# TigreGotico/phoonnx

Hardware: AMD Instinct MI355X
Metric: audio samples/sec (22.05 kHz), batch-32 256-phoneme utterances (higher is better)
Workload: dtype f32 (f16x3 split: fp32 operands as two fp16 planes, three MFMA products, fp32 accumulate)

## Files before the change

### include/vitsmi.h

```cpp
#ifndef VITSMI_H
#define VITSMI_H

#include <stddef.h>
#include <stdint.h>

#ifdef __cplusplus
extern "C" {
#endif

typedef struct vits_handle vits_handle;

enum {
    VITS_OK = 0,
    VITS_E_IO = -1,
    VITS_E_FORMAT = -2,
    VITS_E_ARG = -3,
    VITS_E_DEVICE = -4,
    VITS_E_NOMEM = -5,
    VITS_E_RANGE = -6
};

#define VITS_MAX_DIMS 4


// ... 192 lines not shown
    int cin, cout, k, dil, t;
} vits_launch_record;
int vits_launch_records(vits_handle *h, vits_launch_record *buf, int n);

void *vits_stream(vits_handle *h);


int vits_test_conv1d(int device_id, const float *x, int B, int Cin, int T, const float *w, const float *bias,
                     int Cout, int K, int dil, int pad_l, int flags, float slope, float *out);
int vits_bench_conv1d(int device_id, int B, int Cin, int Cout, int T, int K, int dil, int hint, int iters,
                      int cfg_override, int ck_override, float *ms_out);
int vits_test_conv_transpose1d(int device_id, const float *x, int B, int Cin, int T, const float *w,
                               const float *bias, int Cout, int K, int stride, float *out);
int vits_test_conv1d_sx(int device_id, const float *x, int B, int Cin, int T, const float *w, const float *bias,
                        int Cout, int K, int dil, int pad_l, int flags, float slope, float *out);
int vits_test_conv1d_sx_planar(int device_id, const float *x, int B, int Cin, int T, const float *w, const float *bias,
                               int Cout, int K, int dil, int flags, const int64_t *lens, const float *old, int row_split,
                               int pl_rows, float *out, float *planes_out);
long long vits_test_set_sx_small_max(long long wgs);
int vits_test_conv1d_sx_gate(int device_id, const float *x, int B, int Cin, int T, const float *w, const float *bias,
                             const float *bias_b, int Cout, int K, int dil, int flags, float *out);
int vits_test_conv_transpose1d_sx(int device_id, const float *x, int B, int Cin, int T, const float *w,
                                  const float *bias, int Cout, int K, int stride, float *out);
int vits_bench_conv1d_sx(int device_id, int B, int Cin, int Cout, int T, int K, int dil, int dbg, int iters,
                         float *ms_out);
int vits_test_conv_pair_sx(int device_id, const float *x, int B, int C, int T, const float *w1, const float *b1,
                           const float *w2, const float *b2, int K, int dil1, int dil2, int chain, float slope, float *out,
                           float *ms_out);
int vits_test_attention(int device_id, const float *qkv, int B, int C, int T, int n_heads, const float *rel_k,
                        const float *rel_v, int window, const int64_t *lens, float *out);
int vits_test_attention16(int device_id, const float *qkv, int B, int C, int T, int n_heads, const float *rel_k,
                          const float *rel_v, int window, const int64_t *lens, float *out, uint16_t *out_planes, int kernel,
                          int reps, float *ms_out);

int vits_test_resample(int device_id, const float *x, const int64_t *lens, int B, int S, int in_rate, int out_rate, float *y,
                       int64_t S_out);
int vits_test_resample_pieces(int device_id, const float *x, const int64_t *lens, int B, int S, int in_rate, int out_rate,
                              int piece_samples, float *y, int64_t S_out, int64_t *ranges, int max_ranges);

int vits_test_durations(int device_id, const float *logw, const int64_t *dur, const int64_t *lens, int B, int T, float length_scale,
                        const float *rows, const float *token_rate, float *w_ceil, int32_t *cum, int32_t *y_len);
int vits_test_expand_prior(int device_id, const float *m_logs, int B, int C, int T, const int32_t *cum, const int64_t *lens,
                           const int32_t *y_len, int F, const float *noise, int64_t noise_stride, int noise_frames,
                           float noise_scale, const float *rows, const uint64_t *seeds, float *z_p);
int vits_test_fill_normal(int device_id, int64_t n, uint64_t seed, uint64_t stream_id, float *out);
int vits_test_fill_normal_rows(int device_id, int B, int channels, int T, const uint64_t *seeds, uint32_t stream, const float *rows,
// ... 47 lines not shown
```

### phoonnx_amd/_ffi.py

```python
import ctypes as C
import os

import numpy as np

from . import audio_encoding

_HERE = os.path.dirname(os.path.abspath(__file__))
_LIB = None

VITS_MAX_DIMS = 4


class VitsNoise(C.Structure):
    _fields_ = [("noise_dp", C.c_void_p), ("noise_z", C.c_void_p), ("noise_z_stride", C.c_int64),
                ("seed", C.c_uint64)]


class VitsOutput(C.Structure):
    _fields_ = [("data", C.POINTER(C.c_float)), ("dims", C.c_int64 * 4), ("y_lengths", C.POINTER(C.c_int64))]


class VitsStats(C.Structure):
    _fields_ = [("conv_flops", C.c_double), ("conv_bytes", C.c_double), ("dec_flops", C.c_double),
                ("dec_bytes", C.c_double), ("flow_flops", C.c_double), ("enc_flops", C.c_double),
# ... 40 lines not shown
class VitsStreamFormat(C.Structure):
    _fields_ = [("encoding", C.c_int32), ("ref_peak", C.c_void_p), ("volume", C.c_void_p)]


ENCODINGS = {name: (code, audio_encoding.DTYPES[name]) for code, name in enumerate(audio_encoding.ENCODINGS)}


CHUNK_FN = C.CFUNCTYPE(C.c_int, C.c_void_p, C.POINTER(C.c_float), C.c_int, C.c_int64, C.c_int64, C.c_int64)

ENC_CHUNK_FN = C.CFUNCTYPE(C.c_int, C.c_void_p, C.c_void_p, C.c_int, C.c_int64, C.c_int64, C.c_int64, C.POINTER(C.c_int32),
                           C.POINTER(C.c_float), C.c_int64)

VITS_E_RANGE = -6


EXPORTS = [
    "vits_open", "vits_open_with_arena", "vits_open_host", "vits_open_layout", "vits_open_opts", "vits_close",
    "vits_run_chunked", "vits_run_vocoder_chunked", "vits_last_error", "vits_num_inputs",
    "vits_input_name", "vits_meta", "vits_hparam", "vits_arena_bytes", "vits_arena_host", "vits_arena_device",
    "vits_run", "vits_free_output", "vits_run_device", "vits_sync", "vits_last_y_lengths", "vits_last_pcm16", "vits_run_vocoder",
    "vits_tap",
    "vits_set_timing", "vits_set_tails", "vits_reserve", "vits_get_stats", "vits_stream", "vits_test_conv1d", "vits_test_conv_transpose1d",
    "vits_test_attention", "vits_test_attention16", "vits_bench_conv1d", "vits_test_conv1d_sx", "vits_test_conv1d_sx_planar", "vits_test_conv1d_sx_gate", "vits_test_set_sx_small_max",
    "vits_test_conv_transpose1d_sx",
    "vits_bench_conv1d_sx", "vits_test_conv_pair_sx", "vits_fetch_output", "vits_run_async", "vits_host_alloc", "vits_host_free",
    "vits_launch_records", "vits_run_async_rows", "vits_run_device_rows", "vits_run_chunked_rows",
    "vits_run_async_ctl", "vits_run_chunked_ctl", "vits_last_durations",
    "vits_set_output_rate", "vits_last_sample_counts", "vits_resample_plan", "vits_test_resample", "vits_test_resample_pieces",
    "vits_test_durations", "vits_test_expand_prior", "vits_test_fill_normal", "vits_test_fill_normal_rows", "vits_test_post_conv",
    "vits_delivery_plan", "vits_deliver", "vits_test_deliver",
    "vits_trim_range", "vits_delivery_plan_trimmed", "vits_deliver_trimmed", "vits_test_deliver_trimmed",
    "vits_loudness_filter", "vits_loudness_gate", "vits_level_gain", "vits_delivery_plan_leveled", "vits_deliver_leveled",
    "vits_test_loudness_blocks", "vits_test_deliver_leveled",
    "vits_run_chunked_enc", "vits_run_vocoder_chunked_enc", "vits_test_stream_pack",
    "vits_test_layernorm", "vits_test_dds", "vits_test_cf_pre", "vits_test_rqs_inverse", "vits_test_ea_logw",
]


G2P_EXPORTS = ["g2p_open", "g2p_close", "g2p_last_error", "g2p_hparam", "g2p_num_outputs", "g2p_output_name", "g2p_bucket",
               "g2p_run", "g2p_generate", "g2p_generate_batch", "g2p_test_forced_steps", "g2p_test_linear", "g2p_test_step"]


def lib_path():
    return os.environ.get("VITSMI_LIB") or os.path.join(_HERE, "libvitsmi.so")


def load():
# ... 93 lines not shown
    lib.vits_tap.argtypes = [vp, C.c_char_p, vp, C.c_size_t, i64p]
    lib.vits_set_timing.argtypes = [vp, C.c_int]
    lib.vits_set_tails.argtypes = [vp, C.c_int]
    lib.vits_reserve.argtypes = [vp, C.c_int, C.c_int, C.c_int]
    lib.vits_get_stats.argtypes = [vp, C.POINTER(VitsStats)]
    lib.vits_stream.argtypes = [vp]
    lib.vits_stream.restype = vp
    lib.vits_fetch_output.argtypes = [vp, vp, C.c_size_t, C.c_size_t]
    lib.vits_host_alloc.argtypes = [C.c_size_t]
    lib.vits_host_alloc.restype = vp
    lib.vits_host_free.argtypes = [vp]
    lib.vits_host_free.restype = None
    lib.vits_launch_records.argtypes = [vp, C.POINTER(VitsLaunchRecord), C.c_int]
    lib.vits_test_conv1d.argtypes = [C.c_int, vp, C.c_int, C.c_int, C.c_int, vp, vp, C.c_int, C.c_int, C.c_int,
                                     C.c_int, C.c_int, C.c_float, vp]
    lib.vits_test_conv_transpose1d.argtypes = [C.c_int, vp, C.c_int, C.c_int, C.c_int, vp, vp, C.c_int, C.c_int,
                                               C.c_int, vp]
    lib.vits_test_attention.argtypes = [C.c_int, vp, C.c_int, C.c_int, C.c_int, C.c_int, vp, vp, C.c_int, vp, vp]
    lib.vits_test_attention16.argtypes = [C.c_int, vp, C.c_int, C.c_int, C.c_int, C.c_int, vp, vp, C.c_int, vp, vp, vp,
                                          C.c_int, C.c_int, f32p]
    lib.vits_bench_conv1d.argtypes = [C.c_int] * 11 + [f32p]
    lib.vits_test_conv1d_sx.argtypes = lib.vits_test_conv1d.argtypes
    lib.vits_test_conv_transpose1d_sx.argtypes = lib.vits_test_conv_transpose1d.argtypes
    lib.vits_test_conv1d_sx_planar.argtypes = [C.c_int, vp, C.c_int, C.c_int, C.c_int, vp, vp, C.c_int, C.c_int, C.c_int, C.c_int,
                                               vp, vp, C.c_int, C.c_int, vp, vp]
    lib.vits_test_set_sx_small_max.argtypes = [C.c_longlong]
    lib.vits_test_set_sx_small_max.restype = C.c_longlong
    lib.vits_test_conv1d_sx_gate.argtypes = [C.c_int, vp, C.c_int, C.c_int, C.c_int, vp, vp, vp, C.c_int, C.c_int, C.c_int, C.c_int, vp]
    lib.vits_bench_conv1d_sx.argtypes = [C.c_int] * 9 + [f32p]
    lib.vits_test_conv_pair_sx.argtypes = [C.c_int, vp, C.c_int, C.c_int, C.c_int, vp, vp, vp, vp, C.c_int, C.c_int,
                                           C.c_int, C.c_int, C.c_float, vp, f32p]
    lib.g2p_open.argtypes = [C.c_char_p, C.c_int, C.POINTER(vp)]
    lib.g2p_close.argtypes = [vp]
    lib.g2p_close.restype = None
    lib.g2p_last_error.argtypes = [vp]
    lib.g2p_last_error.restype = C.c_char_p
    lib.g2p_hparam.argtypes = [vp, C.c_char_p, i64p]
    lib.g2p_num_outputs.argtypes = [vp]
    lib.g2p_output_name.argtypes = [vp, C.c_int]
    lib.g2p_output_name.restype = C.c_char_p
    lib.g2p_bucket.argtypes = [vp, C.c_int, C.c_int]
    lib.g2p_run.argtypes = [vp, vp, C.c_int, vp, vp, C.c_int, vp]
    lib.g2p_generate.argtypes = [vp, vp, C.c_int, C.c_int, C.c_int64, C.c_int64, vp, C.POINTER(C.c_int)]
    lib.g2p_generate_batch.argtypes = [vp, vp, vp, C.c_int, C.c_int, C.c_int64, C.c_int64, vp, vp]
    lib.g2p_test_forced_steps.argtypes = [vp, vp, vp, C.c_int, vp, C.c_int, vp]
    lib.g2p_test_linear.argtypes = [C.c_int, C.c_int, vp, vp, C.c_int, vp, C.c_int, C.c_int, vp, C.c_int64, C.c_int64, C.c_int, vp]
# ... 12 lines not shown
```

### phoonnx_amd/csrc/conv_sx_engine.hip.hpp

```cpp
#pragma once
#include <hip/hip_runtime.h>
#include <stdint.h>

#include <cstdio>
#include <cstdlib>
#include <string>
#include <utility>

#include "conv_engine.hip.hpp"
#include "conv_geom.hpp"

#ifndef SX_CFG0_WIDE
#define SX_CFG0_WIDE 0
#endif
#ifndef SX16_SPREAD
#define SX16_SPREAD 0
#endif
#ifndef SX16_PRIO
#define SX16_PRIO 0
#endif
#ifndef SX16_ABL
#define SX16_ABL 0
#endif
#ifndef SX16_NA_SMALL
// ... 377 lines not shown
            for (int n = 0; n < NW; n++)
#pragma unroll
                for (int r = 0; r < 16; r++) acc[m][n][r] = 0.f;
    }
    constexpr bool PRE = RAWIN && EPI >= 0 && (EPI & SX_RES_EARLY) != 0;
    constexpr int NRND_ = MW * (NW / 2);
    f32x4 pre[PRE ? NRND_ : 1][2][4];

    if constexpr (S16) {
    constexpr int HPS = MW;
    constexpr int NQ = NW;
    struct AHalf {
        u32x4 f[2][NPL];
    };
    f32x4 c16[MW][2][NW][2];
#pragma unroll
    for (int m = 0; m < MW; m++)
#pragma unroll
        for (int aa = 0; aa < 2; aa++)
#pragma unroll
            for (int n = 0; n < NW; n++)
#pragma unroll
                for (int bb = 0; bb < 2; bb++) c16[m][aa][n][bb] = f32x4{0.f, 0.f, 0.f, 0.f};
    const int S = a.nchunks * K, H = S * HPS;
    int ztap = -1;
    if constexpr (MW == 1 && WN == 1) {
        if (a.zt_p >= 0 && a.ups > 1) {
            const int blk = (mt * BM + wm * 32) >> 5;
            ztap = __builtin_amdgcn_readfirstlane(((blk % a.ups) + a.zt_p) / a.ups == 0 ? 2 : 0);
        }
    }
    bool zskip = false;
    const uint32_t voff0 = (uint32_t)lane * 16u;
    auto load_ah = [&](AHalf &f, int hs) __attribute__((always_inline)) {
        const int st = hs / HPS, m = hs - st * HPS;
        const uint64_t pa = reinterpret_cast<uint64_t>(wbase) + (uint64_t)((int64_t)st * STEPBYTES + m * BLKBYTES);
        const char *sb = reinterpret_cast<const char *>(((uint64_t)(uint32_t)__builtin_amdgcn_readfirstlane((unsigned)(pa >> 32)) << 32) |
                                                        (uint64_t)(uint32_t)__builtin_amdgcn_readfirstlane((unsigned)pa));
        if constexpr (H1) {
            f.f[0][0] = global_read128<0>(voff0, sb);
            f.f[1][0] = global_read128<1024>(voff0, sb);
        } else {
            f.f[0][0] = global_read128<0>(voff0, sb);
            f.f[0][1] = global_read128<1024>(voff0, sb);
            f.f[1][0] = global_read128<2048>(voff0, sb);
            f.f[1][1] = global_read128<3072>(voff0, sb);
        }
    };
    constexpr int NAL = 2 * NPL;
    const uint32_t b_lane = lds0 + (uint32_t)((lane >> 4) * RS + wn * (NW * 32) + (lane & 15)) * 16u;
    const uint32_t plane_b = (uint32_t)(4 * RS) * 16u;
    u32x4 bq[2][2][NPL];
    auto load_bq = [&](auto BUF, auto Q, uint32_t bb0) __attribute__((always_inline)) {
        constexpr int bf = decltype(BUF)::value, q = decltype(Q)::value;
        if constexpr ((SX16_ABL & 2) != 0) return;
        bq[bf][0][0] = ds_read128<q * 512>(bb0);
        if constexpr (!H1) bq[bf][0][1] = ds_read128<q * 512>(bb0 + plane_b);
        bq[bf][1][0] = ds_read128<q * 512 + 256>(bb0);
        if constexpr (!H1) bq[bf][1][1] = ds_read128<q * 512 + 256>(bb0 + plane_b);
    };
    auto wait_bq = [&]() __attribute__((always_inline)) {
        if constexpr (H1) asm volatile("s_waitcnt lgkmcnt(2)" ::: "memory");
        else asm volatile("s_waitcnt lgkmcnt(4)" ::: "memory");
    };
    auto mma_q = [&](const AHalf &f, auto M, auto BUF, auto Q) __attribute__((always_inline)) {
        constexpr int m = decltype(M)::value, bf = decltype(BUF)::value, q = decltype(Q)::value;
        if constexpr ((SX16_ABL & 1) != 0) return;
        if constexpr (MW == 1 && WN == 1) {
            if (zskip) return;
        }
        if constexpr (SX16_PRIO) __builtin_amdgcn_s_setprio(1);
        if constexpr (H1) {
#pragma unroll
            for (int aa = 0; aa < 2; aa++)
#pragma unroll
                for (int bb = 0; bb < 2; bb++)
                    c16[m][aa][q][bb] = __builtin_amdgcn_mfma_f32_16x16x32_f16(__builtin_bit_cast(f16x8, f.f[aa][0]),
                                                                               __builtin_bit_cast(f16x8, bq[bf][bb][0]),
                                                                               c16[m][aa][q][bb], 0, 0, 0);
        } else
#pragma unroll
        for (int c = 0; c < 3; c++)
#pragma unroll
            for (int aa = 0; aa < 2; aa++)
#pragma unroll
                for (int bb = 0; bb < 2; bb++) {
                    const f16x8 ga = c == 0 ? __builtin_bit_cast(f16x8, f.f[aa][NPL - 1])
                                            : (c == 1 ? __builtin_bit_cast(f16x8, f.f[aa][0]) * (_Float16)0.00048828125f
                                                      : __builtin_bit_cast(f16x8, f.f[aa][0]));
                    c16[m][aa][q][bb] = __builtin_amdgcn_mfma_f32_16x16x32_f16(ga, __builtin_bit_cast(f16x8, bq[bf][bb][c == 1 ? NPL - 1 : 0]),
                                                                               c16[m][aa][q][bb], 0, 0, 0);
                }
        if constexpr (SX16_PRIO) __builtin_amdgcn_s_setprio(0);
// ... 3 lines not shown
            case 0: asm volatile("s_waitcnt vmcnt(0)" ::: "memory"); break;
            case 1: asm volatile("s_waitcnt vmcnt(1)" ::: "memory"); break;
            case 2: asm volatile("s_waitcnt vmcnt(2)" ::: "memory"); break;
            case 3: asm volatile("s_waitcnt vmcnt(3)" ::: "memory"); break;
            case 4: asm volatile("s_waitcnt vmcnt(4)" ::: "memory"); break;
            case 5: asm volatile("s_waitcnt vmcnt(5)" ::: "memory"); break;
            case 6: asm volatile("s_waitcnt vmcnt(6)" ::: "memory"); break;
            case 7: asm volatile("s_waitcnt vmcnt(7)" ::: "memory"); break;
            case 8: asm volatile("s_waitcnt vmcnt(8)" ::: "memory"); break;
            case 9: asm volatile("s_waitcnt vmcnt(9)" ::: "memory"); break;
            case 10: asm volatile("s_waitcnt vmcnt(10)" ::: "memory"); break;
            case 11: asm volatile("s_waitcnt vmcnt(11)" ::: "memory"); break;
            default: asm volatile("s_waitcnt vmcnt(12)" ::: "memory"); break;
        }
    };
    const std::integral_constant<int, 0> I0{};
    const std::integral_constant<int, 1> I1{};
    constexpr int NA = NW == 2 ? SX16_NA_SMALL : 2;
    static_assert(NA >= 2 && NA <= 4, "");
    issue_x(0, 0);
    AHalf ab[NA];
    static_for<NA - 1>([&](auto I) {
        constexpr int i = decltype(I)::value;
        if (i < H) load_ah(ab[i], i);
    });
    int chunk = 0, tap = 0;
    int iss[NA - 1], xct[NA - 1];
#pragma unroll
    for (int j = 0; j < NA - 1; j++) {
        iss[j] = NAL;
        xct[j] = 0;
    }
    int a_since_x = NAL * (NA - 1);
    auto half_step = [&](AHalf &fc, AHalf &fload, auto M, int hs) __attribute__((always_inline)) {
        constexpr int m = decltype(M)::value;
        const bool chunk_start = m == 0 && tap == 0;
        zskip = tap == ztap;
        int allow = xct[NA - 2];
#pragma unroll
        for (int j = 0; j < NA - 2; j++) allow += iss[j];
        if (chunk_start && a_since_x < allow) allow = a_since_x;
        if (__builtin_expect(allow == 0, 1)) asm volatile("s_waitcnt vmcnt(0) lgkmcnt(15)" ::: "memory");
        else wait_vm16(allow);
        const bool more_x = chunk + 1 < a.nchunks;
        if (chunk_start && !(SX16_ABL & 4)) {
            __builtin_amdgcn_s_barrier();
        }
        __builtin_amdgcn_sched_barrier(0);
#pragma unroll
        for (int j = NA - 2; j > 0; j--) {
            iss[j] = iss[j - 1];
            xct[j] = xct[j - 1];
        }
        iss[0] = xct[0] = 0;
        if (hs + NA - 1 < H && !(SX_NOA && hs > 0)) {
            load_ah(fload, hs + NA - 1);
            iss[0] = NAL;
            a_since_x += NAL;
        }
        const bool do_x = chunk_start && more_x;
        if (do_x) {
            if constexpr (!SX16_SPREAD) issue_x(chunk + 1, ((chunk + 1) & 1) * XB);
            iss[0] += nx_issued;
            xct[0] = nx_issued;
            a_since_x = 0;
        }
        __builtin_amdgcn_sched_barrier(0);
        const uint32_t bb0 = b_lane + (uint32_t)(chunk & 1) * XB + (uint32_t)(tap * a.dil) * 16u;
        const bool last_of_chunk = m == HPS - 1 && tap == K - 1;
        const uint32_t bnext = m == HPS - 1 ? bb0 + (uint32_t)a.dil * 16u : bb0;
        if (chunk_start) load_bq(I0, I0, bb0);
        static_for<NQ>([&](auto Q) {
            constexpr int q = decltype(Q)::value;
            constexpr int bf = q & 1;
            __builtin_amdgcn_sched_barrier(0);
            if constexpr (q + 1 < NQ) {
                load_bq(std::integral_constant<int, (q + 1) & 1>{}, std::integral_constant<int, q + 1>{}, bb0);
                wait_bq();
            } else {
                if (!last_of_chunk && hs + 1 < H) {
                    load_bq(std::integral_constant<int, NQ & 1>{}, I0, bnext);
                    wait_bq();
                } else
                    asm volatile("s_waitcnt lgkmcnt(0)" ::: "memory");
            }
            __builtin_amdgcn_sched_barrier(0);
            mma_q(fc, M, std::integral_constant<int, bf>{}, Q);
            if constexpr (SX16_SPREAD) {
                if (do_x) {
                    __builtin_amdgcn_sched_barrier(0);
                    const char *cb = reinterpret_cast<const char *>(xb) + (int64_t)(XG * (chunk + 1)) * T * 16;
                    const uint32_t xoff = ((chunk + 1) & 1) * XB;
#pragma unroll
                    for (int it = q; it < MAXIT; it += NQ)
                        if (it < nit && xok[it])
                            lds_dma<16, kSxXAux>(cb + xoffs[it], reinterpret_cast<float *>(lds_sx + xoff + (it * 256 + wave * 64) * 16));
                }
            }
        });
        __builtin_amdgcn_sched_barrier(0);
        if (m == HPS - 1 && ++tap == K) {
            tap = 0;
            chunk++;
        }
    };
    static_assert(NQ % 2 == 0, "the first quarter of a half-step always lands in quarter buffer 0");
    constexpr int U = NA * HPS / (NA % HPS == 0 ? HPS : 1) / (HPS % NA == 0 && NA != HPS ? NA : 1);
    static_assert(U % NA == 0 && U % HPS == 0, "one period of weight sets and row halves");
    int hs = 0;
    for (; hs + U <= H; hs += U)
        static_for<U>([&](auto I) {
            constexpr int i = decltype(I)::value;
            half_step(ab[i % NA], ab[(i + NA - 1) % NA], std::integral_constant<int, i % HPS>{}, hs + i);
        });
    __builtin_amdgcn_sched_barrier(0);
    asm volatile("s_waitcnt lgkmcnt(0)" ::: "memory");
    __builtin_amdgcn_sched_barrier(0);
    static_for<U - 1>([&](auto I) {
        constexpr int i = decltype(I)::value;
        if (hs + i < H) half_step(ab[i % NA], ab[(i + NA - 1) % NA], std::integral_constant<int, i % HPS>{}, hs + i);
    });
#pragma unroll
    for (int m = 0; m < MW; m++)
#pragma unroll
        for (int n = 0; n < NW; n++)
// ... 336 lines not shown
            }
            return;
        }
    }
    const int u = a.ups, Cr = a.Cr, Tout = T * u, CGo = Cr >> 3;
    float *rawb = a.out_raw + (int64_t)b * a.raw_bstride;
    uint16_t *plb = a.out_pl + (int64_t)b * a.pl_bstride;
    const float *resb = a.res + (int64_t)b * a.raw_bstride;
    const uint16_t *resplb = a.res_pl + (int64_t)b * a.pl_bstride;
    const float unsl = a.res_unslope;
    const bool respl = H1 || (EPI >= 0 ? (EPI & SX_RES_PL) != 0 : a.res_pl != nullptr);
    const bool res_epi = (flags & EPI_RES) && !PRE;
    const float *addp = res_epi ? resb : rawb;
    const bool has_add = res_epi || (flags & EPI_ACC);
    const bool two_adds = res_epi && (flags & EPI_ACC);
    const float oslope = a.oslope, oslope2 = a.oslope2, rdiv = a.div;
    const float wsc = a.wscale;
    const int64_t plane_elems = (int64_t)CGo * Tout * 8;
    const float *biasp = a.bias ? a.bias : a.zeros;
    const int b_on = a.bias ? 1 : 0;
    constexpr int NRND = MW * (NW / 2);
    constexpr bool PIPE = EPI >= 0 && ((EPI & EPI_RES) != 0 && !PRE) != ((EPI & EPI_ACC) != 0);
    f32x4 adb[PIPE ? 2 : 1][2][4], ad2[2][4];
    auto geom = [&](int m, int n, int &co0, int &r, int &t) {
        const int row0 = mt * BM + (wm * MW + m) * 32;
        r = u == 1 ? 0 : (row0 >> 5) % u;
        co0 = u == 1 ? row0 : (row0 / (32 * u)) * 32;
        t = t0 + (wn * NW + n) * 32 + l31;
    };
    auto cell_at = [&](int co0, int r, int t, int q) -> int64_t {
        return ((int64_t)((co0 >> 3) + q) * Tout + (t * u + r)) * 8 + 4 * hi;
    };
    auto issue_adds = [&](auto R, auto P) {
        constexpr int rr = decltype(R)::value, pp = decltype(P)::value;
        constexpr int m = rr / (NW / 2), n0 = (rr % (NW / 2)) * 2;
#pragma unroll
        for (int j = 0; j < 2; j++) {
            int co0, r, t;
            geom(m, n0 + j, co0, r, t);
            const int tl = t < T ? t : T - 1;
#pragma unroll
            for (int q = 0; q < 4; q++) {
                const int64_t c = cell_at(co0, r, tl, q);
                if (respl) {
                    if (res_epi) {
                        float o4[4];
                        if constexpr (H1) {
                            unact4h(*reinterpret_cast<const u32x2 *>(resplb + c), unsl, o4);
                        } else {
                            float h0[4], h1[4];
                            unact4h(*reinterpret_cast<const u32x2 *>(resplb + c), 1.f, h0);
                            unact4h(*reinterpret_cast<const u32x2 *>(resplb + plane_elems + c), 1.f, h1);
#pragma unroll
                            for (int e = 0; e < 4; e++) {
                                const float v = __builtin_fmaf(h1[e], 1.f / 2048.f, h0[e]);
                                o4[e] = v < 0.f ? v * unsl : v;
                            }
                        }
                        adb[pp][j][q] = f32x4{o4[0], o4[1], o4[2], o4[3]};
                    } else if (has_add)
                        adb[pp][j][q] = *reinterpret_cast<const f32x4 *>(rawb + c);
                } else if (has_add)
                    adb[pp][j][q] = *reinterpret_cast<const f32x4 *>(addp + c);
                if (two_adds) ad2[j][q] = *reinterpret_cast<const f32x4 *>(rawb + c);
            }
        }
    };
    if constexpr (PIPE) issue_adds(std::integral_constant<int, 0>{}, std::integral_constant<int, 0>{});
    static_for<NRND>([&](auto R) {
        constexpr int rr = decltype(R)::value;
        constexpr int m = rr / (NW / 2), n0 = (rr % (NW / 2)) * 2;
        constexpr int pp = PIPE ? (rr & 1) : 0;
        if constexpr (PIPE) {
            if constexpr (rr + 1 < NRND) issue_adds(std::integral_constant<int, rr + 1>{}, std::integral_constant<int, (rr + 1) & 1>{});
        } else
            issue_adds(R, std::integral_constant<int, 0>{});
        int co0m, rm, tm;
        geom(m, n0, co0m, rm, tm);
        const int row0 = mt * BM + (wm * MW + m) * 32;
        f32x4 bq[4];
#pragma unroll
        for (int q = 0; q < 4; q++) {
            bq[q] = *reinterpret_cast<const f32x4 *>(biasp + (row0 + 8 * q + 4 * hi) * b_on);
            if (flags & SX_HAS_BIASB)
                bq[q] += *reinterpret_cast<const f32x4 *>(a.bias_b + (int64_t)b * a.bias_b_stride + co0m + 8 * q + 4 * hi);
        }
#pragma unroll
        for (int j = 0; j < 2; j++) {
            constexpr int dummy = 0;
            (void)dummy;
            const int n = n0 + j;
            int co0, r, t;
            geom(m, n, co0, r, t);
            if (t >= TV) continue;
#pragma unroll
            for (int q = 0; q < 4; q++) {
                const int64_t cell = cell_at(co0, r, t, q);
                f32x4 v;
#pragma unroll
                for (int e = 0; e < 4; e++) {
                    if constexpr (F16) v[e] = __builtin_fmaf(acc[m][n][4 * q + e], wsc, bq[q][e]);
                    else v[e] = acc[m][n][4 * q + e] + bq[q][e];
                }
                if constexpr (PRE) v += pre[rr][j][q];
                if (has_add) v += adb[pp][j][q];
                if (two_adds) v += ad2[j][q];
                if (flags & EPI_DIV) {
#pragma unroll
                    for (int e = 0; e < 4; e++) v[e] = v[e] / rdiv;
                }
                if (flags & SX_HAS_RAW) {
                    f32x4 o = v;
                    if (flags & SX_RAW_ACT) {
#pragma unroll
                        for (int e = 0; e < 4; e++) o[e] = fmaxf(v[e], v[e] * oslope);
                    }
                    *reinterpret_cast<f32x4 *>(rawb + cell) = o;
                }
                if (flags & SX_HAS_PL) {
                    f32x4 o = v;
                    if (flags & SX_PL_ACT) {
#pragma unroll
                        for (int e = 0; e < 4; e++) o[e] = fmaxf(v[e], v[e] * oslope2);
                    }
                    unsigned wa[3], wb[3];
                    if constexpr (H1) {
                        wa[0] = cvt1h_pair_pk(o[0], o[1], pk);
                        wb[0] = cvt1h_pair_pk(o[2], o[3], pk);
                    } else if constexpr (F16) {
                        split2h_pair_pk(o[0], o[1], wa[0], wa[1], pk);
                        split2h_pair_pk(o[2], o[3], wb[0], wb[1], pk);
                    } else {
                        split3_pair(o[0], o[1], wa[0], wa[1], wa[2]);
                        split3_pair(o[2], o[3], wb[0], wb[1], wb[2]);
                    }
#pragma unroll
                    for (int pl = 0; pl < NPL; pl++)
                        *reinterpret_cast<u32x2 *>(plb + pl * plane_elems + cell) = u32x2{wa[pl], wb[pl]};
                }
            }
        }
    });
    if constexpr (F16) {
        if (a.peak) {
            if constexpr (S16) sx_publish_peak_at(a.peak, (int)blockIdx.x, pk, reinterpret_cast<float *>(lds_sx));
            else sx_publish_peak(a.peak, (int)blockIdx.x, pk);
        }
    }
}


template <int MW, int NW, int WM, int WN, int EPI = -1, bool PROF = false, bool RAWIN = false, int NP = 6, int SH = 32>
inline hipError_t launch_conv_sx_k(const SxArgs &a, dim3 grid, size_t lds, hipStream_t stream) {
    static std::atomic<uint64_t> attr_done{0};
    auto kern = conv_sx_kernel<MW, NW, WM, WN, EPI, PROF, RAWIN, NP, SH>;
    if (hipError_t e = sx_allow_big_lds(reinterpret_cast<const void *>(kern), attr_done); e != hipSuccess) return e;
    if (g_launch_name_on)
        snprintf(g_launch_name, sizeof g_launch_name, "conv_sx_kernel<%d, %d, %d, %d, %d, %s, %s, %d, %d>", MW, NW, WM, WN, EPI,
                 PROF ? "true" : "false", RAWIN ? "true" : "false", NP, SH);
    kern<<<grid, 256, lds, stream>>>(a);
    return hipGetLastError();
}

constexpr int kSxEpiPlanes = SX_HAS_PL | SX_PL_ACT;
constexpr int kSxEpiUp = SX_HAS_RAW | SX_HAS_PL | SX_PL_ACT;
// ... 315 lines not shown
```

### phoonnx_amd/csrc/vitsmi.hip

```cpp
#include <climits>
#include <hip/hip_runtime.h>

#include <cmath>
#include <cstdarg>
#include <chrono>
#include <cstdio>
#include <cstring>
#include <mutex>
#include <string>
#include <vector>

#include "../../include/vitsmi.h"
#include "conv_geom.hpp"
#include "conv_sx_engine.hip.hpp"
#include "conv_sx_pair.hip.hpp"
#include "conv_sx_pair16.hip.hpp"
#include "attention16.hip.hpp"
#include "conv_sx_small.hip.hpp"
#include "delivery.hip.hpp"
#include "kernels.hip.hpp"
#include "loudness.hip.hpp"
#include "model.hpp"
#include "resample.hip.hpp"
#include "stream_pack.hip.hpp"
// ... 3372 lines not shown
        ms_out[0] = ms;
        ms_out[1] = (float)d.cfg;
        ms_out[2] = (float)d.CK;
    }
    return VITS_OK;
}

int vits_test_conv_transpose1d(int device_id, const float *x, int B, int Cin, int T, const float *w, const float *bias,
                               int Cout, int K, int stride, float *out) {
    if (int rc = test_dev(device_id)) return rc;
    ConvDesc d;
    std::vector<float> arena;
    { std::string e = pack_test_convT(w, bias, Cin, Cout, K, stride, &d, &arena); if (!e.empty()) return fail(nullptr, VITS_E_ARG, "%s", e.c_str()); }
    return run_test_conv(d, arena, x, B, T, 0, 0.f, out, (size_t)B * Cout * T * stride, (int64_t)Cout * T * stride);
}

static TestPack sx_test_pack(SxPack::Planes planes = SxPack::F16X2) {
    TestPack o;
    o.sx.planes = planes;
    return o;
}

static int run_test_conv_sx(const ConvDesc &d, const std::vector<float> &arena, const float *x, int B, int T, int flags,
                            float slope, float *out) {
    const int Cr = d.Cout / d.ups, To = T * d.ups;
    const size_t nx = (size_t)B * d.Cin * T, no = (size_t)B * Cr * To;
    if ((flags & 4) && (d.Cin != d.Cout || d.ups != 1)) return fail(nullptr, VITS_E_ARG, "residual test needs Cin == Cout");
    std::vector<float> xa;
    if (d.h1 && (flags & 8)) {
        xa.resize(nx);
        for (size_t i = 0; i < nx; i++) xa[i] = x[i] >= 0.f ? x[i] : x[i] * slope;
        x = xa.data();
    }
    DevBufs D;
    float *dA = D.up(arena.data(), arena.size());
    float *dx = D.up(x, nx, 16);
    uint16_t *dxp = D.alloc<uint16_t>(nx * 3, 16);
    float *draw = D.fill<float>(no, 0, 16);
    uint16_t *dop = D.fill<uint16_t>(no * 3, 0, 16);
    float *dout = D.alloc<float>(no, 16);
    float *dres = D.alloc<float>(nx, 16);
    TCHECK(D.err);
    sx_split_planes_kernel<<<dim3((T + 255) / 256, d.Cin / 8, B), 256>>>(dx, (int64_t)d.Cin * T, T, nullptr, dxp, d.Cin, T,
                                                                         d.h1 ? 2 : (d.f16 ? 1 : 0));
    sx_block_kernel<<<dim3((T + 255) / 256, d.Cin / 8, B), 256>>>(dx, (int64_t)d.Cin * T, T, nullptr, dres, d.Cin, T);
    SxArgs a = sx_args(d, dA, dA, T);
    a.xp = reinterpret_cast<const u32x4 *>(dxp);
    a.xr = dres;
    a.islope = (flags & 8) ? slope : 1.f;
    a.out_raw = (flags & 128) ? nullptr : draw;
    a.out_pl = dop;
    a.oslope = 1.f;
    a.oslope2 = (flags & 1) ? slope : 1.f;
    if (flags & 4) {
        if (d.h1) {
            a.res_pl = dxp;
            a.res_unslope = (flags & 8) ? 1.f / slope : 1.f;
        } else
            a.res = dres;
        a.flags |= EPI_RES;
    }
    const int nprod = d.h1 ? 1 : (d.f16 ? 2 : 6);
    if (flags & 256) {
        if (!conv_sx_small_ok(a, d.rawin, nprod)) return fail(nullptr, VITS_E_ARG, "arguments not taken by the short-launch kernel");
        TCHECK(launch_conv_sx_small(a, B, d.cfg, nullptr));
    } else
        TCHECK(launch_conv_sx(a, d.cfg, B, nullptr, d.rawin, nprod));
    sx_unblock_kernel<<<dim3((To + 255) / 256, Cr / 8, B), 256>>>(draw, (flags & 1) ? dop : nullptr, dout, Cr, To,
                                                                  d.h1 ? 2 : (d.f16 ? 1 : 0));
    TCHECK(hipGetLastError());
    TCHECK(hipDeviceSynchronize());
    TCHECK(download(out, dout, no));
    return VITS_OK;
}

int vits_test_conv1d_sx(int device_id, const float *x, int B, int Cin, int T, const float *w, const float *bias, int Cout,
                        int K, int dil, int pad_l, int flags, float slope, float *out) {
    if (int rc = test_dev(device_id)) return rc;
    ConvDesc d;
    std::vector<float> arena;
    const int prec = (flags >> 4) & 3;
    if (prec == 1) return fail(nullptr, VITS_E_ARG, "precision code 1 (bf16x3) was retired");
    if ((flags & 128) && !(flags & 1)) return fail(nullptr, VITS_E_ARG, "planes-only output is read back from the planes (bit 0)");
    const TestPack o = sx_test_pack(prec == 2 ? SxPack::F16X1 : (prec == 3 ? SxPack::F16X2 : SxPack::BF16X3));
    std::string e = pack_test_conv(w, bias, Cin, Cout, K, dil, pad_l, 3, &d, &arena, o);
    if (!e.empty()) return fail(nullptr, VITS_E_ARG, "%s", e.c_str());
    return run_test_conv_sx(d, arena, x, B, T, flags, slope, out);
}

int vits_test_conv1d_sx_planar(int device_id, const float *x, int B, int Cin, int T, const float *w, const float *bias,
// ... 96 lines not shown
    else a.out_raw = dact;
    if (flags & 1) {
        if (!conv_sx_small_ok(a, false, 2)) return fail(nullptr, VITS_E_ARG, "arguments not taken by the short-launch kernel");
        TCHECK(launch_conv_sx_small(a, B, d.cfg, nullptr));
    } else
        TCHECK(launch_conv_sx(a, d.cfg == 0 ? 3 : d.cfg, B, nullptr, false, 2, d.cfg));
    if (flags & 2) sx_unblock_kernel<<<dim3((T + 255) / 256, H / 8, B), 256>>>(nullptr, dpl, dact, H, T, 1);
    TCHECK(hipGetLastError());
    TCHECK(hipDeviceSynchronize());
    TCHECK(download(out, dact, no));
    return VITS_OK;
}

int vits_test_conv_transpose1d_sx(int device_id, const float *x, int B, int Cin, int T, const float *w, const float *bias,
                                  int Cout, int K, int stride, float *out) {
    if (int rc = test_dev(device_id)) return rc;
    ConvDesc d;
    std::vector<float> arena;
    const bool f16 = stride < 0;
    if (f16) stride = -stride;
    std::string e = pack_test_convT(w, bias, Cin, Cout, K, stride, &d, &arena, true, sx_test_pack(f16 ? SxPack::F16X2 : SxPack::BF16X3));
    if (!e.empty()) return fail(nullptr, VITS_E_ARG, "%s", e.c_str());
    return run_test_conv_sx(d, arena, x, B, T, 0, 0.f, out);
}

int vits_test_conv_pair_sx(int device_id, const float *x, int B, int C, int T, const float *w1, const float *b1,
                           const float *w2, const float *b2, int K, int dil1, int dil2, int chain, float slope, float *out,
                           float *ms_out) {
    if (int rc = test_dev(device_id)) return rc;
    const int kern = (chain >> 1) & 3;
    const bool from_plane = (chain & 8) != 0;
    chain &= 1;
    const bool h1 = kern == 2;
    ConvDesc d1, d2;
    std::vector<float> arena;
    TestPack o = sx_test_pack(h1 ? SxPack::F16X1 : SxPack::F16X2);
    o.sx.force16 = kern && !h1;
    std::string e = pack_test_conv(w1, b1, C, C, K, dil1, dil1 * (K - 1) / 2, 3, &d1, &arena, o);
    if (e.empty()) e = pack_test_conv(w2, b2, C, C, K, dil2, dil2 * (K - 1) / 2, 3, &d2, &arena, o);
    if (!e.empty()) return fail(nullptr, VITS_E_ARG, "%s", e.c_str());
    const size_t n = (size_t)B * C * T;
    DevBufs D;
    if (kern) {
        if (!d1.s16 || !d2.s16 || d1.rawin || !sx_pair16_plan(C, h1 ? 1 : 2, d1.K, d1.dil, d2.K, d2.dil, nullptr))
            return fail(nullptr, VITS_E_ARG, "this conv pair cannot run fused on the 16x16x32 loop (C %d, kernel %d, dilation %d)", C, K, dil1);
        std::vector<float> xa(n);
// ... 894 lines not shown
```

### phoonnx_amd/session.py

```python
import ctypes as C
import time
from dataclasses import dataclass
from typing import Dict, List, Optional, Sequence

import numpy as np

from . import _ffi


class SessionError(RuntimeError):
    """Raised for every failure of the engine (onnxruntime raises its own
    InvalidArgument/RuntimeException at voice.py:374; callers there do not catch either)."""


class RangeError(SessionError):
    """VITS_E_RANGE: the f16x3 generator arithmetic met an activation beyond the range of its fp16 operand planes
    (|x| > 65504) or a non-finite value.  The engine reports this instead of returning clamped audio; `MiSession`
    (range_fallback=True, the default) then reopens the voice with the bf16x6 arithmetic (fp32 range) and repeats the
    call, so user code only sees this when the fallback is switched off or impossible (borrowed weight arena)."""


class _PinnedPool:

    def __init__(self, keep_bytes=2 << 30):
# ... 1456 lines not shown
    if rc != 0:
        raise SessionError(_ffi.last_error(None))
    if dbg & 16:
        return float(res[0]), int(res[1]), [float(v) for v in res[3:8]] + [float(res[2])]
    return float(res[0]), int(res[1])


def test_conv_transpose1d(x, w, bias, stride, device_id=0, sx=False):
    lib = _ffi.load()
    x = np.ascontiguousarray(x, np.float32)
    w = np.ascontiguousarray(w, np.float32)
    B, Cin, T = x.shape
    _, Cout, K = w.shape
    b = None if bias is None else np.ascontiguousarray(bias, np.float32)
    out = np.empty((B, Cout, T * stride), np.float32)
    fn = lib.vits_test_conv_transpose1d_sx if sx else lib.vits_test_conv_transpose1d
    rc = fn(device_id, _ffi.ptr(x), B, Cin, T, _ffi.ptr(w), _ffi.ptr(b), Cout, K, -stride if sx == "f16" else stride,
            _ffi.ptr(out))
    if rc != 0:
        raise SessionError(_ffi.last_error(None))
    return out


def test_attention16(qkv, n_heads, rel_k, rel_v, lens, device_id=0, kernel=1, planes=False, reps=0):
    lib = _ffi.load()
    qkv = np.ascontiguousarray(qkv, np.float32)
    B, C3, T = qkv.shape
    Cc = C3 // 3
    rel_k = np.ascontiguousarray(rel_k, np.float32)
    rel_v = np.ascontiguousarray(rel_v, np.float32)
    window = (rel_k.shape[0] - 1) // 2
    lens = np.ascontiguousarray(lens, np.int64)
    out = np.empty((B, Cc, T), np.float32)
    opl = np.empty((B, 3, Cc // 8, T, 8), np.uint16) if planes else None
    ms = (C.c_float * 1)()
    rc = lib.vits_test_attention16(device_id, _ffi.ptr(qkv), B, Cc, T, n_heads, _ffi.ptr(rel_k), _ffi.ptr(rel_v), window,
                                   _ffi.ptr(lens), _ffi.ptr(out), _ffi.ptr(opl) if planes else None, int(kernel), int(reps), ms)
    if rc != 0:
        raise SessionError(_ffi.last_error(None))
    res = (out,)
    if planes:
        res += (opl,)
    if reps > 0:
        res += (float(ms[0]),)
    return res[0] if len(res) == 1 else res

# ... 417 lines not shown
```

Before: 146.8 million.

## Stage transposed-conv epilogue through LDS and trim zero-tap loop for upsample

```diff
diff --git a/include/vitsmi.h b/include/vitsmi.h
--- a/include/vitsmi.h
+++ b/include/vitsmi.h
@@ -238,6 +238,9 @@
                              const float *bias_b, int Cout, int K, int dil, int flags, float *out);
 int vits_test_conv_transpose1d_sx(int device_id, const float *x, int B, int Cin, int T, const float *w,
                                   const float *bias, int Cout, int K, int stride, float *out);
+int vits_test_conv_transpose1d_sx_opt(int device_id, const float *x, int B, int Cin, int T, const float *w,
+                                      const float *bias, int Cout, int K, int stride, int flags, float slope,
+                                      const int *ends, char *kernel_out, int kernel_cap, float *out);
 int vits_bench_conv1d_sx(int device_id, int B, int Cin, int Cout, int T, int K, int dil, int dbg, int iters,
                          float *ms_out);
 int vits_test_conv_pair_sx(int device_id, const float *x, int B, int C, int T, const float *w1, const float *b1,
diff --git a/phoonnx_amd/_ffi.py b/phoonnx_amd/_ffi.py
--- a/phoonnx_amd/_ffi.py
+++ b/phoonnx_amd/_ffi.py
@@ -86,7 +86,7 @@
     "vits_tap",
     "vits_set_timing", "vits_set_tails", "vits_reserve", "vits_get_stats", "vits_stream", "vits_test_conv1d", "vits_test_conv_transpose1d",
     "vits_test_attention", "vits_test_attention16", "vits_bench_conv1d", "vits_test_conv1d_sx", "vits_test_conv1d_sx_planar", "vits_test_conv1d_sx_gate", "vits_test_set_sx_small_max",
-    "vits_test_conv_transpose1d_sx",
+    "vits_test_conv_transpose1d_sx", "vits_test_conv_transpose1d_sx_opt",
     "vits_bench_conv1d_sx", "vits_test_conv_pair_sx", "vits_fetch_output", "vits_run_async", "vits_host_alloc", "vits_host_free",
     "vits_launch_records", "vits_run_async_rows", "vits_run_device_rows", "vits_run_chunked_rows",
     "vits_run_async_ctl", "vits_run_chunked_ctl", "vits_last_durations",
@@ -226,6 +226,8 @@
     lib.vits_bench_conv1d.argtypes = [C.c_int] * 11 + [f32p]
     lib.vits_test_conv1d_sx.argtypes = lib.vits_test_conv1d.argtypes
     lib.vits_test_conv_transpose1d_sx.argtypes = lib.vits_test_conv_transpose1d.argtypes
+    lib.vits_test_conv_transpose1d_sx_opt.argtypes = [C.c_int, vp, C.c_int, C.c_int, C.c_int, vp, vp, C.c_int, C.c_int, C.c_int,
+                                                      C.c_int, C.c_float, vp, C.c_char_p, C.c_int, vp]
     lib.vits_test_conv1d_sx_planar.argtypes = [C.c_int, vp, C.c_int, C.c_int, C.c_int, vp, vp, C.c_int, C.c_int, C.c_int, C.c_int,
                                                vp, vp, C.c_int, C.c_int, vp, vp]
     lib.vits_test_set_sx_small_max.argtypes = [C.c_longlong]
diff --git a/phoonnx_amd/csrc/conv_sx_engine.hip.hpp b/phoonnx_amd/csrc/conv_sx_engine.hip.hpp
--- a/phoonnx_amd/csrc/conv_sx_engine.hip.hpp
+++ b/phoonnx_amd/csrc/conv_sx_engine.hip.hpp
@@ -423,15 +423,18 @@
             for (int n = 0; n < NW; n++)
 #pragma unroll
                 for (int bb = 0; bb < 2; bb++) c16[m][aa][n][bb] = f32x4{0.f, 0.f, 0.f, 0.f};
-    const int S = a.nchunks * K, H = S * HPS;
-    int ztap = -1;
-    if constexpr (MW == 1 && WN == 1) {
-        if (a.zt_p >= 0 && a.ups > 1) {
+    constexpr bool LT = MW == 1 && WN == 1;
+    int tap0 = 0, tapN = K;
+    if constexpr (LT) {
+        if (a.zt_p >= 0 && a.ups > 1 && K == 3) {
             const int blk = (mt * BM + wm * 32) >> 5;
-            ztap = __builtin_amdgcn_readfirstlane(((blk % a.ups) + a.zt_p) / a.ups == 0 ? 2 : 0);
-        }
-    }
-    bool zskip = false;
+            const bool z2 = __builtin_amdgcn_readfirstlane(((blk % a.ups) + a.zt_p) / a.ups == 0 ? 1 : 0) != 0;
+            tap0 = z2 ? 0 : 1;
+            tapN = z2 ? 2 : 3;
+        }
+    }
+    const int KL = tapN - tap0;
+    const int H = a.nchunks * KL * HPS;
     const uint32_t voff0 = (uint32_t)lane * 16u;
     auto load_ah = [&](AHalf &f, int hs) __attribute__((always_inline)) {
         const int st = hs / HPS, m = hs - st * HPS;
@@ -448,6 +451,18 @@
             f.f[1][1] = global_read128<3072>(voff0, sb);
         }
     };
+    int la_st = tap0, la_tap = tap0;
+    auto next_ah = [&](AHalf &f, int hs) __attribute__((always_inline)) {
+        if constexpr (LT) {
+            load_ah(f, la_st);
+            la_st++;
+            if (++la_tap == tapN) {
+                la_tap = tap0;
+                la_st += K - KL;
+            }
+        } else
+            load_ah(f, hs);
+    };
     constexpr int NAL = 2 * NPL;
     const uint32_t b_lane = lds0 + (uint32_t)((lane >> 4) * RS + wn * (NW * 32) + (lane & 15)) * 16u;
     const uint32_t plane_b = (uint32_t)(4 * RS) * 16u;
@@ -467,9 +482,6 @@
     auto mma_q = [&](const AHalf &f, auto M, auto BUF, auto Q) __attribute__((always_inline)) {
         constexpr int m = decltype(M)::value, bf = decltype(BUF)::value, q = decltype(Q)::value;
         if constexpr ((SX16_ABL & 1) != 0) return;
-        if constexpr (MW == 1 && WN == 1) {
-            if (zskip) return;
-        }
         if constexpr (SX16_PRIO) __builtin_amdgcn_s_setprio(1);
         if constexpr (H1) {
 #pragma unroll
@@ -519,9 +531,9 @@
     AHalf ab[NA];
     static_for<NA - 1>([&](auto I) {
         constexpr int i = decltype(I)::value;
-        if (i < H) load_ah(ab[i], i);
+        if (i < H) next_ah(ab[i], i);
     });
-    int chunk = 0, tap = 0;
+    int chunk = 0, tap = tap0;
     int iss[NA - 1], xct[NA - 1];
 #pragma unroll
     for (int j = 0; j < NA - 1; j++) {
@@ -531,8 +543,7 @@
     int a_since_x = NAL * (NA - 1);
     auto half_step = [&](AHalf &fc, AHalf &fload, auto M, int hs) __attribute__((always_inline)) {
         constexpr int m = decltype(M)::value;
-        const bool chunk_start = m == 0 && tap == 0;
-        zskip = tap == ztap;
+        const bool chunk_start = m == 0 && tap == tap0;
         int allow = xct[NA - 2];
 #pragma unroll
         for (int j = 0; j < NA - 2; j++) allow += iss[j];
@@ -551,7 +562,7 @@
         }
         iss[0] = xct[0] = 0;
         if (hs + NA - 1 < H && !(SX_NOA && hs > 0)) {
-            load_ah(fload, hs + NA - 1);
+            next_ah(fload, hs + NA - 1);
             iss[0] = NAL;
             a_since_x += NAL;
         }
@@ -564,7 +575,7 @@
         }
         __builtin_amdgcn_sched_barrier(0);
         const uint32_t bb0 = b_lane + (uint32_t)(chunk & 1) * XB + (uint32_t)(tap * a.dil) * 16u;
-        const bool last_of_chunk = m == HPS - 1 && tap == K - 1;
+        const bool last_of_chunk = m == HPS - 1 && tap == tapN - 1;
         const uint32_t bnext = m == HPS - 1 ? bb0 + (uint32_t)a.dil * 16u : bb0;
         if (chunk_start) load_bq(I0, I0, bb0);
         static_for<NQ>([&](auto Q) {
@@ -596,8 +607,8 @@
             }
         });
         __builtin_amdgcn_sched_barrier(0);
-        if (m == HPS - 1 && ++tap == K) {
-            tap = 0;
+        if (m == HPS - 1 && ++tap == tapN) {
+            tap = tap0;
             chunk++;
         }
     };
@@ -980,16 +991,16 @@
     constexpr int NRND = MW * (NW / 2);
     constexpr bool PIPE = EPI >= 0 && ((EPI & EPI_RES) != 0 && !PRE) != ((EPI & EPI_ACC) != 0);
     f32x4 adb[PIPE ? 2 : 1][2][4], ad2[2][4];
-    auto geom = [&](int m, int n, int &co0, int &r, int &t) {
+    auto geom = [&](int m, int n, int &co0, int &r, int &t) __attribute__((always_inline)) {
         const int row0 = mt * BM + (wm * MW + m) * 32;
         r = u == 1 ? 0 : (row0 >> 5) % u;
         co0 = u == 1 ? row0 : (row0 / (32 * u)) * 32;
         t = t0 + (wn * NW + n) * 32 + l31;
     };
-    auto cell_at = [&](int co0, int r, int t, int q) -> int64_t {
+    auto cell_at = [&](int co0, int r, int t, int q) __attribute__((always_inline)) -> int64_t {
         return ((int64_t)((co0 >> 3) + q) * Tout + (t * u + r)) * 8 + 4 * hi;
     };
-    auto issue_adds = [&](auto R, auto P) {
+    auto issue_adds = [&](auto R, auto P) __attribute__((always_inline)) {
         constexpr int rr = decltype(R)::value, pp = decltype(P)::value;
         constexpr int m = rr / (NW / 2), n0 = (rr % (NW / 2)) * 2;
 #pragma unroll
@@ -1024,11 +1035,87 @@
             }
         }
     };
+    constexpr bool LROUTE = S16 && MW == 1 && WN == 1 &&
+                            (EPI < 0 || (EPI & ~SX_PL_ACT) == SX_HAS_PL || (EPI & ~SX_RAW_ACT) == SX_HAS_RAW);
+    constexpr int LTS = 68;
+    constexpr uint32_t l_plane = 16u * LTS * 16u;
+    uint32_t l_raw = 0, l_need = 0;
+    bool via = false, l_dbl = false;
+    if constexpr (LROUTE) {
+        if (u > 1 && (u & 3) == 0 && a.zt_p >= 0 && !(flags & SX_WN_RMW)) {
+            l_raw = (flags & SX_HAS_RAW) ? 16u * LTS * 32u : 0u;
+            l_need = l_raw + ((flags & SX_HAS_PL) ? NPL * l_plane : 0u);
+            via = l_need <= a.lds_bytes;
+            l_dbl = 2 * l_need <= a.lds_bytes;
+        }
+    }
+    const uint32_t lw_raw = (uint32_t)((wm * LTS + l31) * 32 + hi * 16);
+    const uint32_t lw_pl = l_raw + (uint32_t)((wm * LTS + l31) * 16 + hi * 8);
+    auto store_runs = [&](int rr, uint32_t lbuf) __attribute__((always_inline)) {
+        const int blk0 = mt * (BM / 32);
+        const int cg0 = (blk0 / u) * 4, r0 = blk0 % u;
+        auto place = [&](int c, int &row, int &tt, int64_t &off) __attribute__((always_inline)) -> bool {
+            const int q = c >> 8, p = c & 3;
+            tt = (c & 255) >> 2;
+            row = q * 4 + p;
+            const int t = t0 + rr * 64 + tt;
+            off = ((int64_t)(cg0 + q) * Tout + ((int64_t)t * u + r0 + p)) * 8;
+            return t < TV;
+        };
+        if (flags & SX_HAS_PL) {
+            u32x4 v[4][NPL];
+#pragma unroll
+            for (int k = 0; k < 4; k++) {
+                int row, tt;
+                int64_t off;
+                place(k * 256 + tid, row, tt, off);
+#pragma unroll
+                for (int pl = 0; pl < NPL; pl++)
+                    v[k][pl] = *reinterpret_cast<const u32x4 *>(lds_sx + lbuf + l_raw + pl * l_plane + (uint32_t)(row * LTS + tt) * 16u);
+            }
+#pragma unroll
+            for (int k = 0; k < 4; k++) {
+                int row, tt;
+                int64_t off;
+                if (place(k * 256 + tid, row, tt, off)) {
+#pragma unroll
+                    for (int pl = 0; pl < NPL; pl++) *reinterpret_cast<u32x4 *>(plb + pl * plane_elems + off) = v[k][pl];
+                }
+            }
+        }
+        if (flags & SX_HAS_RAW) {
+#pragma unroll
+            for (int k0 = 0; k0 < 8; k0 += 4) {
+                f32x4 v[4];
+#pragma unroll
+                for (int k = 0; k < 4; k++) {
+                    const int c = (k0 + k) * 256 + tid;
+                    int row, tt;
+                    int64_t off;
+                    place(c >> 1, row, tt, off);
+                    v[k] = *reinterpret_cast<const f32x4 *>(lds_sx + lbuf + (uint32_t)(row * LTS + tt) * 32u + (uint32_t)(c & 1) * 16u);
+                }
+#pragma unroll
+                for (int k = 0; k < 4; k++) {
+                    const int c = (k0 + k) * 256 + tid;
+                    int row, tt;
+                    int64_t off;
+                    if (place(c >> 1, row, tt, off)) *reinterpret_cast<f32x4 *>(rawb + off + 4 * (c & 1)) = v[k];
+                }
+            }
+        }
+    };
     if constexpr (PIPE) issue_adds(std::integral_constant<int, 0>{}, std::integral_constant<int, 0>{});
-    static_for<NRND>([&](auto R) {
+    auto rounds = [&](auto VIA) __attribute__((always_inline)) {
+    constexpr bool via_ = decltype(VIA)::value;
+    static_for<NRND>([&](auto R) __attribute__((always_inline)) {
         constexpr int rr = decltype(R)::value;
         constexpr int m = rr / (NW / 2), n0 = (rr % (NW / 2)) * 2;
         constexpr int pp = PIPE ? (rr & 1) : 0;
+        const uint32_t lbuf = (via_ && l_dbl && (rr & 1)) ? l_need : 0u;
+        if constexpr (via_) {
+            if (rr == 0 || !l_dbl) __syncthreads();
+        }
         if constexpr (PIPE) {
             if constexpr (rr + 1 < NRND) issue_adds(std::integral_constant<int, rr + 1>{}, std::integral_constant<int, (rr + 1) & 1>{});
         } else
@@ -1073,7 +1160,8 @@
 #pragma unroll
                         for (int e = 0; e < 4; e++) o[e] = fmaxf(v[e], v[e] * oslope);
                     }
-                    *reinterpret_cast<f32x4 *>(rawb + cell) = o;
+                    if constexpr (via_) *reinterpret_cast<f32x4 *>(lds_sx + lbuf + lw_raw + (uint32_t)((q * 4 * LTS + j * 32) * 32)) = o;
+                    else *reinterpret_cast<f32x4 *>(rawb + cell) = o;
                 }
                 if (flags & SX_HAS_PL) {
                     f32x4 o = v;
@@ -1093,12 +1181,27 @@
                         split3_pair(o[2], o[3], wb[0], wb[1], wb[2]);
                     }
 #pragma unroll
-                    for (int pl = 0; pl < NPL; pl++)
-                        *reinterpret_cast<u32x2 *>(plb + pl * plane_elems + cell) = u32x2{wa[pl], wb[pl]};
-                }
-            }
+                    for (int pl = 0; pl < NPL; pl++) {
+                        if constexpr (via_)
+                            *reinterpret_cast<u32x2 *>(lds_sx + lbuf + lw_pl + pl * l_plane + (uint32_t)((q * 4 * LTS + j * 32) * 16)) =
+                                u32x2{wa[pl], wb[pl]};
+                        else
+                            *reinterpret_cast<u32x2 *>(plb + pl * plane_elems + cell) = u32x2{wa[pl], wb[pl]};
+                    }
+                }
+            }
+        }
+        if constexpr (via_) {
+            __syncthreads();
+            store_runs(rr, lbuf);
         }
     });
+    };
+    if constexpr (LROUTE) {
+        if (via) rounds(std::true_type{});
+        else rounds(std::false_type{});
+    } else
+        rounds(std::false_type{});
     if constexpr (F16) {
         if (a.peak) {
             if constexpr (S16) sx_publish_peak_at(a.peak, (int)blockIdx.x, pk, reinterpret_cast<float *>(lds_sx));
diff --git a/phoonnx_amd/csrc/vitsmi.hip b/phoonnx_amd/csrc/vitsmi.hip
--- a/phoonnx_amd/csrc/vitsmi.hip
+++ b/phoonnx_amd/csrc/vitsmi.hip
@@ -3418,7 +3418,7 @@
 }
 
 static int run_test_conv_sx(const ConvDesc &d, const std::vector<float> &arena, const float *x, int B, int T, int flags,
-                            float slope, float *out) {
+                            float slope, float *out, const int *ends = nullptr, char *kernel_out = nullptr, int kernel_cap = 0) {
     const int Cr = d.Cout / d.ups, To = T * d.ups;
     const size_t nx = (size_t)B * d.Cin * T, no = (size_t)B * Cr * To;
     if ((flags & 4) && (d.Cin != d.Cout || d.ups != 1)) return fail(nullptr, VITS_E_ARG, "residual test needs Cin == Cout");
@@ -3436,6 +3436,7 @@
     uint16_t *dop = D.fill<uint16_t>(no * 3, 0, 16);
     float *dout = D.alloc<float>(no, 16);
     float *dres = D.alloc<float>(nx, 16);
+    int *dends = ends ? D.up(ends, (size_t)B) : nullptr;
     TCHECK(D.err);
     sx_split_planes_kernel<<<dim3((T + 255) / 256, d.Cin / 8, B), 256>>>(dx, (int64_t)d.Cin * T, T, nullptr, dxp, d.Cin, T,
                                                                          d.h1 ? 2 : (d.f16 ? 1 : 0));
@@ -3456,12 +3457,24 @@
             a.res = dres;
         a.flags |= EPI_RES;
     }
+    if (dends) a.rag = SxRagged{dends, 0, 1};
     const int nprod = d.h1 ? 1 : (d.f16 ? 2 : 6);
+    const bool name_was_on = g_launch_name_on;
+    if (kernel_out) {
+        g_launch_name_on = true;
+        g_launch_name[0] = 0;
+    }
+    hipError_t le;
     if (flags & 256) {
         if (!conv_sx_small_ok(a, d.rawin, nprod)) return fail(nullptr, VITS_E_ARG, "arguments not taken by the short-launch kernel");
-        TCHECK(launch_conv_sx_small(a, B, d.cfg, nullptr));
+        le = launch_conv_sx_small(a, B, d.cfg, nullptr);
     } else
-        TCHECK(launch_conv_sx(a, d.cfg, B, nullptr, d.rawin, nprod));
+        le = launch_conv_sx(a, d.cfg, B, nullptr, d.rawin, nprod);
+    if (kernel_out) {
+        if (kernel_cap > 0) std::snprintf(kernel_out, (size_t)kernel_cap, "%s", g_launch_name);
+        g_launch_name_on = name_was_on;
+    }
+    TCHECK(le);
     sx_unblock_kernel<<<dim3((To + 255) / 256, Cr / 8, B), 256>>>(draw, (flags & 1) ? dop : nullptr, dout, Cr, To,
                                                                   d.h1 ? 2 : (d.f16 ? 1 : 0));
     TCHECK(hipGetLastError());
@@ -3604,6 +3617,20 @@
     std::string e = pack_test_convT(w, bias, Cin, Cout, K, stride, &d, &arena, true, sx_test_pack(f16 ? SxPack::F16X2 : SxPack::BF16X3));
     if (!e.empty()) return fail(nullptr, VITS_E_ARG, "%s", e.c_str());
     return run_test_conv_sx(d, arena, x, B, T, 0, 0.f, out);
+}
+
+int vits_test_conv_transpose1d_sx_opt(int device_id, const float *x, int B, int Cin, int T, const float *w, const float *bias,
+                                      int Cout, int K, int stride, int flags, float slope, const int *ends, char *kernel_out,
+                                      int kernel_cap, float *out) {
+    if (int rc = test_dev(device_id)) return rc;
+    if (flags & ~3) return fail(nullptr, VITS_E_ARG, "unknown flag bits");
+    ConvDesc d;
+    std::vector<float> arena;
+    TestPack o = sx_test_pack((flags & 2) ? SxPack::F16X1 : SxPack::F16X2);
+    o.sx.force16 = !(flags & 2);
+    std::string e = pack_test_convT(w, bias, Cin, Cout, K, stride, &d, &arena, true, o);
+    if (!e.empty()) return fail(nullptr, VITS_E_ARG, "%s", e.c_str());
+    return run_test_conv_sx(d, arena, x, B, T, (flags & 1) ? (1 | 128) : 0, slope, out, ends, kernel_out, kernel_cap);
 }
 
 int vits_test_conv_pair_sx(int device_id, const float *x, int B, int C, int T, const float *w1, const float *b1,
diff --git a/phoonnx_amd/session.py b/phoonnx_amd/session.py
--- a/phoonnx_amd/session.py
+++ b/phoonnx_amd/session.py
@@ -1502,6 +1502,26 @@
     return out
 
 
+def test_conv_transpose1d_sx_opt(x, w, bias, stride, planes_slope=None, single_plane=False, ends=None, device_id=0):
+    lib = _ffi.load()
+    x = np.ascontiguousarray(x, np.float32)
+    w = np.ascontiguousarray(w, np.float32)
+    B, Cin, T = x.shape
+    _, Cout, K = w.shape
+    b = None if bias is None else np.ascontiguousarray(bias, np.float32)
+    e = None if ends is None else np.ascontiguousarray(ends, np.int32)
+    if e is not None and e.shape != (B,):
+        raise ValueError("ends: one column count per utterance")
+    out = np.empty((B, Cout, T * stride), np.float32)
+    name = C.create_string_buffer(128)
+    rc = lib.vits_test_conv_transpose1d_sx_opt(device_id, _ffi.ptr(x), B, Cin, T, _ffi.ptr(w), _ffi.ptr(b), Cout, K, stride,
+                                               (1 if planes_slope is not None else 0) | (2 if single_plane else 0),
+                                               float(planes_slope or 0.0), _ffi.ptr(e), name, len(name), _ffi.ptr(out))
+    if rc != 0:
+        raise SessionError(_ffi.last_error(None))
+    return out, name.value.decode()
+
+
 def test_attention16(qkv, n_heads, rel_k, rel_v, lens, device_id=0, kernel=1, planes=False, reps=0):
     lib = _ffi.load()
     qkv = np.ascontiguousarray(qkv, np.float32)
```

Result: no change. 147.8 million (median of 6 runs) (+0.6%).
